# drscotthawley/signaltrain

Hardware: AMD Instinct MI355X
Metric: audio-frames/sec (train step) comp_4c 8192-sample windows @ 1/2/4/8 GPUs (higher is better)
Workload: dtype f32; 1 GPU; comp_4c synthetic, 8192-sample windows, batch 256/GPU, fp32 (BASELINE configs[1]); window=8192, frames_per_window=25, global_batch=256, parallelism=dp1

## Files before the change

### signaltrain_amd/csrc/st_api.hip

```cpp
#include <hip/hip_runtime.h>
#include <stdarg.h>
#include <stdio.h>
#include <string.h>
#include <math.h>
#include <mutex>
#include <set>
#include <utility>
#include "st_common.h"
#include "st_gemm.h"
#include "st_gemm_planes.h"
#include "st_gemm_tn.h"
#include "st_gemm16.h"
#include "st_misc.h"
#include "st_ae.h"
#include "st_ae_wide.h"
#include "st_ae_split.h"
#include "st_ae32.h"
#include "st_dp.h"
#include "st_feed.h"

static thread_local char g_err[512] = "";
int st_fail(int code, const char* fmt, ...)
{
    va_list ap; va_start(ap, fmt); vsnprintf(g_err, sizeof(g_err), fmt, ap); va_end(ap);
// ... 130 lines not shown
static int g_dbg = 0;
extern "C" int st_set_debug(int v) { g_dbg = v; return ST_OK; }
namespace sta { extern __device__ unsigned long long g_ae_stage_cycles[32]; }
extern "C" int st_debug_read_stage_cycles(unsigned long long* out32);
static int g_dp_inline = 1;
static int g_ae_save = 1;
static int g_ae_split = -1;
static int g_ae32 = 1;
static int g_pl_bf16 = 0;
static int g_wg_split = 0;
static int g_pl_dgrad = 0;
static int g_pl_shape = 3;
static int g_g16 = 1;
static int g_g16_bk = 64;
static int g_g16_dma = 0;
static int g_g16_abl = 0;
static int g_g16_split = 0;
static int g_nt128 = 1;
static int g_tn128 = 1;
static int g_tn_bk = 32;
static int g_tn_fm = 3;
static int g_g16_crop = 15;
static int g_frs_nt = 1;
static int g_xt = 0;
static const int NORM_E_PARTIALS = 32;
static const int NORM_E_MAX = 4096;
static int g_wide_pair = 1;
static int g_wide_direct = 1;
static int g_wide_dvp = 1;
static int g_nt_mi = 0;
static int g_an_bk = 32;
static int g_bk = 16;
static int g_wg_mode_set(int v);
static int g_wsplit_max = 16, g_wsplit_div = 200, g_an_waves = 4, g_syn_split = 3, g_frs_split = 3, g_wide_fused = 1, g_wsplit_half = 0;
extern "C" int st_set_tuning(int bk)
{
#ifdef ST_DIAG
    if (bk >= 96800 && bk < 96928) { g_g16_abl = bk - 96800; return ST_OK; }
#else
    if ((bk >= 96800 && bk < 96928) || (bk >= 9680 && bk < 9690)) return st_fail(ST_ERR_ARG, "st_set_tuning(%d): timing-only ablation, needs a -DST_DIAG build", bk);
#endif
    if (bk >= 9970 && bk < 9980) { g_wide_direct = bk - 9970; return ST_OK; }
    if (bk >= 9960) { g_wide_pair = bk - 9960; return ST_OK; }
    if (bk >= 9950 && bk < 9960) { g_nt128 = bk - 9950; return ST_OK; }
    if (bk >= 9900) { g_wide_dvp = bk - 9900; return ST_OK; }
    if (bk >= 9800) { g_nt_mi = bk - 9800; return ST_OK; }
    if (bk >= 9700) { g_g16_split = bk - 9700; return ST_OK; }
    if (bk >= 9690 && bk < 9700) { g_g16_dma = bk - 9690; return ST_OK; }
#ifdef ST_DIAG
    if (bk >= 9680 && bk < 9690) { g_g16_abl = bk - 9680; return ST_OK; }
#endif
    if (bk >= 9600) { const int v = bk - 9600; if (v == 32 || v == 64) g_g16_bk = v; else g_g16 = v; return ST_OK; }
    if (bk >= 9560 && bk < 9576) { g_g16_crop = bk - 9560; return ST_OK; }
    if (bk >= 9540 && bk < 9544) { g_tn_fm = bk - 9540; return ST_OK; }
    if (bk >= 9500) { const int v = bk - 9500; if (v == 16 || v == 32) g_tn_bk = v; else g_tn128 = v; return ST_OK; }
    if (bk >= 9400) { g_pl_bf16 = bk - 9400; return ST_OK; }
    if (bk >= 9300) { g_wg_split = bk - 9300; return ST_OK; }
    if (bk >= 9200) { g_pl_dgrad = bk - 9200; return ST_OK; }
    if (bk >= 9100) { g_pl_shape = bk - 9100; return ST_OK; }
    if (bk >= 9000) { g_frs_nt = bk - 9000; return ST_OK; }
    if (bk >= 8100 && bk < 8110) { g_ae32 = bk - 8100; return ST_OK; }
    if (bk == 8300 || bk == 8301) { g_dp_inline = bk - 8300; return ST_OK; }
    if (bk == 8200 || bk == 8201) { g_ae_save = bk - 8200; return ST_OK; }
    if (bk >= 8000) { g_ae_split = bk == 8002 ? -1 : bk - 8000; return ST_OK; }
    if (bk >= 7000) { g_xt = bk - 7000; return ST_OK; }
    if (bk >= 6000) { g_wsplit_half = bk - 6000; return ST_OK; }
    if (bk >= 5000) { g_wide_fused = bk - 5000; return ST_OK; }
    if (bk >= 4000) { g_frs_split = bk - 4000; return (g_frs_split >= 1 && g_frs_split <= 6) ? ST_OK : st_fail(ST_ERR_ARG, "frames split must be 1..6"); }
    if (bk >= 3000) { g_syn_split = bk - 3000; return ST_OK; }
    if (bk >= 2000) { g_an_waves = bk - 2000; return ST_OK; }
    if (bk >= 1000) { g_wsplit_div = bk - 1000; return ST_OK; }
    if (bk >= 200) { g_wsplit_max = bk - 200; return ST_OK; }
    if (bk >= 100) return g_wg_mode_set(bk - 100);
    if (bk != 16 && bk != 32) return st_fail(ST_ERR_ARG, "bk must be 16 or 32"); g_bk = bk; g_an_bk = bk; return ST_OK;
}
#define ST_TUNING_LIST(X) X(g_dbg, 0) X(g_ae_split, -1) X(g_ae_save, 1) X(g_dp_inline, 1) X(g_pl_bf16, 0) X(g_wg_split, 0) X(g_pl_dgrad, 0) X(g_pl_shape, 3) X(g_g16, 1) X(g_g16_bk, 64) X(g_g16_dma, 0) \
    X(g_g16_abl, 0) X(g_g16_split, 0) X(g_nt128, 1) X(g_tn128, 1) X(g_tn_bk, 32) X(g_frs_nt, 1) X(g_xt, 0) X(g_wide_pair, 1) X(g_wide_dvp, 1) X(g_nt_mi, 0) X(g_an_bk, 32) \
    X(g_bk, 16) X(g_wsplit_max, 16) X(g_wsplit_div, 200) X(g_an_waves, 4) X(g_syn_split, 3) X(g_frs_split, 3) X(g_wide_fused, 1) X(g_wsplit_half, 0) X(g_wg_mode, 0) X(g_ae32, 1) X(g_wide_direct, 1) X(g_tn_fm, 3) X(g_g16_crop, 15)
static int g_wg_mode = 0;
extern "C" int st_get_tuning(int* out, int n)
{
    int i = 0;
#define X(v_, d_) if (out && i < n) out[i] = v_; ++i;
    ST_TUNING_LIST(X)
#undef X
    return i;
}
extern "C" int st_tuning_defaults(int* out, int n)
{
    int i = 0;
#define X(v_, d_) if (out && i < n) out[i] = d_; ++i;
    ST_TUNING_LIST(X)
#undef X
    return i;
}
extern "C" int st_reset_tuning(void)
{
#define X(v_, d_) v_ = d_;
    ST_TUNING_LIST(X)
#undef X
    return ST_OK;
}
static inline int gemm_ht(int prec) { return (prec == ST_PREC_BF16 || prec == ST_PREC_BF16_ALL) ? 1 : ((prec == ST_PREC_F16 || prec == ST_PREC_F16_ALL) ? 2 : (prec == ST_PREC_F32X3 ? 3 : 0)); }
static inline int ae_ht(int prec) { return prec == ST_PREC_BF16_ALL ? 1 : (prec == ST_PREC_F16_ALL ? 2 : 0); }
static inline float loss_scale_of(const st_dims* d) { return d->loss_scale > 0.f ? d->loss_scale : 1.0f; }
#define ST_GEMM_BK(BK_, W_, ...) do { const int ht_ = gemm_ht(d->prec); \
// ... 345 lines not shown
    return ola_loss_impl(d, frs, x, y_true, y_hat, dsyn, 0, loss_partial, stream);
}

static int synthesis_dgrad_impl(const st_dims* d, const float* dsyn, bool padded, const float* Sfold, float* dAA, void* stream)
{
    const int KP = st_kp_of(d->F);
    const stg::RowMap ms = synth_live(d);
    const int R = ms.rows(d->B);
    stg::PlainNT bl{Sfold, KP, d->N, d->N, stg::all_frames(1)};
    stg::StoreC ep{dAA, R, KP, KP, (size_t)d->B * d->OT * KP, ms};
    const int ns = R >= 4096 ? 1 : synth_split(R);
    if (padded) {
        stg::FramedNT<true> al{dsyn, d->y, d->H, d->N, R, d->N, 1.0f, ms};
        stg::NTWork wk;
        if (use_nt128(d, R, KP) && stg::ntw_dgrad(wk, ms, d->B, d->H, d->N, d->N, d->y, d->F, KP, ns, num_cus())) {
            const stg::NTRows ra = stg::ntrows_frame_major(dsyn, (unsigned)(d->y + 2 * d->N), (unsigned)d->H, ms, d->B, R);
            const stg::NTRows rb = wk.col_h ? stg::NTRows{Sfold, (unsigned)((KP / 2) * d->N), (unsigned)d->N, stg::rowmap_magic(d->F - 1), d->F - 1, 0, 2 * (d->F - 1)}
                                            : stg::NTRows{Sfold, (unsigned)d->N, 0u, 0u, 1, 0, KP};
            const stg::StoreSlab es{dAA, R, KP, KP, (size_t)d->B * d->OT * KP, stg::frame_major(ms, d->B)};
            ST_TRY(stg::launch_nt128(ra, rb, es, wk, st_stream(stream)));
        }
        else if (R >= 4096) ST_GEMM(4, al, bl, ep, R, KP, d->N, ns, st_stream(stream));
        else if (gemm_ht(d->prec) == 0 && (g_nt_mi & 4)) stg::launch<2, 16, 2>(al, bl, ep, R, KP, d->N, ns, st_stream(stream), g_dbg);
        else ST_GEMM(2, al, bl, ep, R, KP, d->N, ns, st_stream(stream));
    } else {
        stg::FramedNT<false> al{dsyn, d->y, d->H, d->N, R, d->N, 1.0f, ms};
        if (R >= 4096) ST_GEMM(4, al, bl, ep, R, KP, d->N, ns, st_stream(stream)); else ST_GEMM(2, al, bl, ep, R, KP, d->N, ns, st_stream(stream));
    }
    ST_LAUNCHED("synthesis_dgrad");
    return ST_OK;
}
extern "C" int st_synthesis_dgrad(const st_dims* d, const float* dsyn, const float* Sfold, float* dAA, void* stream)
{
    ST_TRY(check_dims(d)); ST_REQ(dsyn && Sfold && dAA, "st_synthesis_dgrad: null pointer");
    return synthesis_dgrad_impl(d, dsyn, false, Sfold, dAA, stream);
}

static bool use_tn128(const st_dims* d, bool padded)
{
    const int ht = gemm_ht(d->prec);
    return g_tn128 && padded && (ht == 0 || (ht == 3 && !g_wg_split)) && d->N % 256 == 0 && g_wg_mode == 0;
}
struct TNFrameMajor { stg::TNOperand a, b; stg::RowMap map; stg::FrameTrim trim; bool on; };
static TNFrameMajor tn_frame_major(const stg::TNOperand& ta, const stg::TNOperand& tb, const stg::RowMap& live, int B, int H, int Ntaps, int pad, int Ls, bool enable)
{
    TNFrameMajor f; f.on = enable && B >= 2 && fm_div_exact(live.Tv * B, B); f.a = ta; f.b = tb; f.map = live; f.trim = stg::FrameTrim{}; f.trim.on = 0;
    if (!f.on) return f;
    f.a = stg::TNOperand{ta.base + (size_t)live.t_lo * ta.S2, ta.S2, ta.S1};
    f.b = stg::TNOperand{tb.base + (size_t)live.t_lo * tb.S2, tb.S2, tb.S1};
    f.map.Tv = B; f.map.t_lo = 0; f.map.magic = stg::rowmap_magic(B); f.map.fm = 0;
    f.trim = stg::frame_trim(live, B, H, Ntaps, pad, Ls);
    return f;
}
static int wgrad_tn128(const st_dims* d, const stg::TNOperand& ta, const stg::TNOperand& tb, const float* zeros, const stg::RowMap& map, int R,
                       float* ws, int ns, stm::NyqJob* nyq, void* stream, const stg::FrameTrim* trim)
{
    const int KP = st_kp_of(d->F);
    const int mh = (d->N / 2) / 128;
    float* part = ws + (size_t)ns * KP * d->N;
    int P = 0;
    const unsigned c0 = (unsigned)(d->F - 1), c1 = (unsigned)(KP / 2 + d->F - 1);
    if (g_tn_bk == 16) ST_TRY((stg::launch_tn128<16>(ta, tb, zeros, map, R, d->N, mh, (unsigned)(KP / 2), d->N, ws, d->N, (size_t)KP * d->N, ns, st_stream(stream), part, c0, c1, &P, trim)));
    else ST_TRY((stg::launch_tn128<32>(ta, tb, zeros, map, R, d->N, mh, (unsigned)(KP / 2), d->N, ws, d->N, (size_t)KP * d->N, ns, st_stream(stream), part, c0, c1, &P, trim)));
    nyq->part = part; nyq->P = P; nyq->on = 1;
    return ST_OK;
}
static int synthesis_wgrad_impl(const st_dims* d, const float* AA, const float* dsyn, bool padded, float* ws,
                                float* gSr, float* gSi, float* norm_partial, void* stream, int* defer_slabs = nullptr, stm::NyqJob* defer_nyq = nullptr)
{
    const int KP = st_kp_of(d->F);
    const stg::RowMap ms = synth_live(d);
    const int R = ms.rows(d->B);
    int ns = wgrad_split_tiles(R, KP, d->N);
    stm::NyqJob nyq{}; nyq.on = 0;
    const stg::TNOperand ta{AA, (unsigned)(d->OT * KP), (unsigned)KP}, tb{dsyn, (unsigned)(d->y + 2 * d->N), (unsigned)d->H};
    if (use_tn128(d, padded) && stg::tn128_fits(ta, tb, dsyn, ms, d->N, d->N, (size_t)d->B * d->OT * KP, (size_t)d->B * (d->y + 2 * d->N))) {
        ns = tn_split(R, d->N);
        const TNFrameMajor fm = tn_frame_major(ta, tb, ms, d->B, d->H, d->N, d->N, d->y, (g_tn_fm & 1) != 0);
        ST_TRY(wgrad_tn128(d, fm.a, fm.b, dsyn, fm.map, R, ws, ns, &nyq, stream, &fm.trim));
    } else {
        stg::PlainTN al{AA, R, KP, KP, ms};
        stg::StoreC ep{ws, KP, d->N, d->N, (size_t)KP * d->N, stg::all_frames(1)};
        if (padded) { stg::FramedTN<true> bl{dsyn, d->y, d->H, d->N, R, d->N, 1.0f, ms}; ST_GEMM_WG(al, bl, ep, KP, d->N, R, ns, st_stream(stream)); }
        else { stg::FramedTN<false> bl{dsyn, d->y, d->H, d->N, R, d->N, 1.0f, ms}; ST_GEMM_WG(al, bl, ep, KP, d->N, R, ns, st_stream(stream)); }
    }
    ST_LAUNCHED("synthesis_wgrad");
    if (defer_slabs) { *defer_slabs = ns; if (defer_nyq) *defer_nyq = nyq; return ST_OK; }
    hipLaunchKernelGGL(stm::wgrad_reduce_kernel, dim3(st_norm_partials(d)), dim3(256), 0, st_stream(stream),
                       ws, ns, gSr, gSi, norm_partial, d->N, d->F, KP, 1, 0, 2 * d->F, (float*)nullptr, nyq);
    ST_LAUNCHED("synthesis_wgrad_reduce");
    return ST_OK;
}
extern "C" int st_synthesis_wgrad(const st_dims* d, const float* AA, const float* dsyn, float* ws,
                                  float* gSr, float* gSi, float* norm_partial, void* stream)
{
    ST_TRY(check_dims(d)); ST_REQ(AA && dsyn && ws && gSr && gSi && norm_partial, "st_synthesis_wgrad: null pointer");
    return synthesis_wgrad_impl(d, AA, dsyn, false, ws, gSr, gSi, norm_partial, stream);
}


static inline int wide_half_type(const st_dims* d, int R) { (void)R; return ae_ht(d->prec); }
extern "C" int st_effective_prec(const st_dims* d)
{
    if (!d) return -1;
    if (ae_is_wide(d) && ae_ht(d->prec) && wide_half_type(d, d->B * (st_kp_of(d->F) / 2)) == 0)
        return d->prec == ST_PREC_BF16_ALL ? ST_PREC_BF16 : ST_PREC_F16;
    return d->prec;
}
#define ST_WGEMM(...) do { if (wide_ht == 1) stg::launch_half<2, 1>(__VA_ARGS__); else if (wide_ht == 2) stg::launch_half<2, 2>(__VA_ARGS__); \
                           else stg::launch<2, 16>(__VA_ARGS__, g_dbg); } while (0)
#define ST_WGEMM_PAIR(A0_, B0_, E0_, A1_, B1_, E1_, M_, N_, K_, NS_, S_) do { \
        if (wide_ht == 1 && g_wide_pair) stg::launch_half_pair<2, 1>(A0_, B0_, E0_, A1_, B1_, E1_, M_, N_, K_, NS_, S_); \
        else if (wide_ht == 2 && g_wide_pair) stg::launch_half_pair<2, 2>(A0_, B0_, E0_, A1_, B1_, E1_, M_, N_, K_, NS_, S_); \
        else { ST_WGEMM(A0_, B0_, E0_, M_, N_, K_, NS_, S_); ST_WGEMM(A1_, B1_, E1_, M_, N_, K_, NS_, S_); } } while (0)
static int ae_wide_fwd(const st_dims* d, const Layout& L, const float* mag, const float* phs, const float* knobs,
                       const float* ae_m, const float* ae_p, float* mag_hat, float* phs_hat, float* AA, float* reg_partial,
// ... 773 lines not shown
    a.nyq = stm::NyqJob{}; a.nyq.on = 0; if (syn_nyq) a.nyq = *syn_nyq;
    a.dG16 = nullptr; a.ht = 0;
    if (w.g16) { a.dG16 = w.dG16; a.ht = gemm_ht(d->prec); a.dG = nullptr; }
    a.norm_e = nullptr;
    if (d->clip_all && a.n_red <= NORM_E_MAX) { a.norm_e = w.norm_e; w.n_norm_e = a.n_red; }
    hipLaunchKernelGGL(stm::post_ae_kernel, dim3(a.n_red + a.n_polar + (syn_slabs > 0 ? st_norm_partials(d) : 0)), dim3(256), 0, st_stream(stream), a);
    ST_LAUNCHED("post_ae");
    return ST_OK;
}
static int backward_p1(const st_dims* d, const Layout& L, const float* params, float* grads,
                       const float* knobs, const float* g_mag_hat, const float* g_mag, float reg_coef, WS& w, void* stream)
{
    int syn_slabs = 0; stm::NyqJob syn_nyq{}; syn_nyq.on = 0;
    ST_TRY(backward_syn(d, L, grads, w, stream, &syn_slabs, &syn_nyq));
    return backward_ae(d, L, params, grads, knobs, g_mag_hat, g_mag, reg_coef, w, stream, syn_slabs, &syn_nyq);
}
static int backward_p2(const st_dims* d, const Layout& L, float* grads, const float* x, WS& w, void* stream, float* stage = nullptr, int stage_bf16 = 0)
{
    (void)x;
    if (w.g16) {
        const stg::RowMap ma = stg::live_frames(d->T, d->H, d->N, d->N, d->L);
        const int R = ma.rows(d->B), KP = st_kp_of(d->F), ns = g16_wsplit(d, R);
        ST_TRY(wgrad16(d, w.dG16, (unsigned)(d->T * KP), w.xp16, (unsigned)(d->L + 2 * d->N), ma, R, w.wg, ns, stream, 0, -1, (g_g16_crop & 8) ? d->L : 0));
        ST_LAUNCHED("analysis_wgrad");
        stm::NyqJob nq{}; nq.on = 0;
        hipLaunchKernelGGL(stm::wgrad_reduce_kernel, dim3(st_norm_partials(d)), dim3(256), 0, st_stream(stream),
                           w.wg, ns, grads + L.offs[0], grads + L.offs[1], w.norm_a, d->N, d->F, KP, 0, 0, 2 * d->F, stage, nq, 0, stage_bf16);
        ST_LAUNCHED("analysis_wgrad_reduce");
        return ST_OK;
    }
    return analysis_wgrad_impl(d, w.dG, w.xp, true, 1.0f, w.wg, grads + L.offs[0], grads + L.offs[1], w.norm_a, stream, -1, stage, stage_bf16);
}
static int analysis_wgrad_half(const st_dims* d, const Layout& L, float* grads, WS& w, int half, float* stage, int stage_bf16, stm::NyqJob* nyq_io, void* stream)
{
    const int KP = st_kp_of(d->F), F = d->F, N = d->N, m0 = half ? KP / 2 : 0;
    const stg::RowMap ma = stg::live_frames(d->T, d->H, d->N, d->N, d->L);
    const int R = ma.rows(d->B);
    const int room = (int)((st_wgrad_ws_floats(d) - (size_t)64 * 2 * N) / ((size_t)KP * N));
    const int per = stm::nyq_blocks(N) / 2;
    int ns;
    const stg::TNOperand ta{w.dG + m0, (unsigned)(d->T * KP), (unsigned)KP}, tb{w.xp, (unsigned)(d->L + 2 * d->N), (unsigned)d->H};
    if (w.g16) {
        const int tiles = ((KP / 2 + 127) / 128) * (N / 128);
        ns = g_g16_split > 0 ? g_g16_split : (2 * num_cus()) / (tiles > 0 ? tiles : 1);
        if (ns > R / 128) ns = R / 128; if (ns > room) ns = room; if (ns < 1) ns = 1;
        ST_TRY(wgrad16(d, w.dG16, (unsigned)(d->T * KP), w.xp16, (unsigned)(d->L + 2 * d->N), ma, R, w.wg, ns, stream, m0, KP / 2, (g_g16_crop & 8) ? d->L : 0));
        if (!half) { *nyq_io = stm::NyqJob{}; nyq_io->on = 0; }
    } else if (use_tn128(d, true) && stg::tn128_fits(ta, tb, w.xp, ma, N / 2, N, (size_t)d->B * d->T * KP, (size_t)d->B * (d->L + 2 * d->N))) {
        const int mh = (N / 2) / 128, tiles = mh * (N / 128);
        ns = num_cus() / (tiles > 0 ? tiles : 1); if (ns > 16) ns = 16; if (ns > R / 64) ns = R / 64; if (ns > room) ns = room; if (ns < 1) ns = 1;
        float* part = w.wg + (size_t)room * KP * N;
        int P = 0;
        const TNFrameMajor fm = tn_frame_major(ta, tb, ma, d->B, d->H, N, N, d->L, (g_tn_fm & 2) != 0);
        if (g_tn_bk == 16) ST_TRY((stg::launch_tn128<16>(fm.a, fm.b, w.xp, fm.map, R, N / 2, mh, (unsigned)(KP / 2), N, w.wg + (size_t)m0 * N, N, (size_t)KP * N, ns, st_stream(stream),
                                                          half ? nullptr : part, (unsigned)(F - 1), (unsigned)(KP / 2 + F - 1), &P, &fm.trim)));
        else ST_TRY((stg::launch_tn128<32>(fm.a, fm.b, w.xp, fm.map, R, N / 2, mh, (unsigned)(KP / 2), N, w.wg + (size_t)m0 * N, N, (size_t)KP * N, ns, st_stream(stream),
                                            half ? nullptr : part, (unsigned)(F - 1), (unsigned)(KP / 2 + F - 1), &P, &fm.trim)));
        if (!half) { nyq_io->part = part; nyq_io->P = P; nyq_io->on = 1; }
    } else {
        ST_LAUNCHED("analysis_wgrad");
        if (!half) { *nyq_io = stm::NyqJob{}; nyq_io->on = 0; }
        return analysis_wgrad_impl(d, w.dG, w.xp, true, 1.0f, w.wg, grads + L.offs[0], grads + L.offs[1], w.norm_a, stream, half, stage, stage_bf16);
    }
    ST_LAUNCHED("analysis_wgrad");
    hipLaunchKernelGGL(stm::wgrad_reduce_kernel, dim3(F + per), dim3(256), 0, st_stream(stream),
                       w.wg, ns, grads + L.offs[0], grads + L.offs[1], w.norm_a, N, F, KP, 0, half * F, F, stage, *nyq_io, half * per, stage_bf16);
    ST_LAUNCHED("analysis_wgrad_reduce");
    return ST_OK;
}
static int backward_impl(const st_dims* d, const Layout& L, const float* params, float* grads, const float* x,
                         const float* knobs, const float* g_mag_hat, const float* g_mag, float reg_coef, WS& w, void* stream)
{
    ST_TRY(backward_p1(d, L, params, grads, knobs, g_mag_hat, g_mag, reg_coef, w, stream));
    return backward_p2(d, L, grads, x, w, stream);
}

extern "C" int st_model_fwd(const st_dims* d, const float* params, const float* x, const float* knobs,
                            float* y_hat, float* mag, float* mag_hat, void* ws, int save_for_backward, void* stream)
{
    Layout L; ST_TRY(make_layout(d, &L));
    ST_REQ(params && x && (knobs || d->K == 0) && ws, "st_model_fwd: null pointer");
    if (!knobs) knobs = params;
    WS w; carve(d, ws, &w);
    return forward_impl(d, L, params, x, knobs, nullptr, y_hat, mag, mag_hat, w, save_for_backward != 0, stream);
}

extern "C" int st_model_bwd(const st_dims* d, const float* params, float* grads, const float* x, const float* knobs,
                            const float* g_y_hat, const float* g_mag_hat, const float* g_mag, void* ws, void* stream)
{
    Layout L; ST_TRY(make_layout(d, &L));
    ST_REQ(params && grads && x && (knobs || d->K == 0) && g_y_hat && ws, "st_model_bwd: null pointer");
    if (!knobs) knobs = params;
    WS w; carve(d, ws, &w);
    ST_TRY(pad_scale(g_y_hat, w.dsyn, d->B, d->y, d->N, 2.0f, stream));
    return backward_impl(d, L, params, grads, x, knobs, g_mag_hat, g_mag, 0.0f, w, stream);
}

__global__ void knob_grad_kernel(const float* __restrict__ Wm, const float* __restrict__ gbm, const float* __restrict__ Wp, const float* __restrict__ gbp,
                                 const int K, float* __restrict__ out)
{
    const int k = threadIdx.x;
    if (k >= K) return;
    float s = 0.f, t = 0.f;
    for (int o = 0; o < 16; ++o) { s += Wm[o * (16 + K) + 16 + k] * gbm[o]; t += Wp[o * (16 + K) + 16 + k] * gbp[o]; }
    out[k] = s + t;
}
extern "C" int st_model_knob_grad(const st_dims* d, const float* params, float* grads_scratch, const float* x, const float* knobs,
                                  const float* g_y_hat, const float* g_mag_hat, const float* g_mag, void* ws, float* g_knobs, void* stream)
{
    Layout L; ST_TRY(make_layout(d, &L));
// ... 620 lines not shown
```

### signaltrain_amd/csrc/st_gemm_tn.h

```cpp
#pragma once
#include "st_gemm.h"

namespace stg {

struct TNJob {
    const float* base;
    unsigned a0, b0;
    unsigned SA1, SA2, SB1, SB2;
    unsigned magic; int Tv, t_lo;
    int K;
    unsigned zero;
    int mh; unsigned mstride;
    float* nyq_out; unsigned nyq_c0, nyq_c1; int nyq_P, Nc, nsplit;
    int trim, fB; unsigned char fa[64], fb[64];
};
struct FrameTrim { int on, B; unsigned char fa[64], fb[64]; };
static inline FrameTrim frame_trim(const RowMap& live, int B, int H, int Ntaps, int pad, int Ls)
{
    FrameTrim f; f.on = (Ntaps % 128 == 0 && Ntaps / 128 <= 64 && live.Tv <= 255) ? 1 : 0; f.B = B;
    for (int j = 0; j < 64; ++j) { f.fa[j] = 0; f.fb[j] = (unsigned char)(live.Tv <= 255 ? live.Tv : 255); }
    if (!f.on) return f;
    for (int j = 0; j < Ntaps / 128; ++j) {
        const int n0 = 128 * j;
        int a = 0, b = live.Tv;
        while (a < b && H * (live.t_lo + a) + n0 + 127 < pad) ++a;
        while (b > a && H * (live.t_lo + b - 1) + n0 >= pad + Ls) --b;
        f.fa[j] = (unsigned char)a; f.fb[j] = (unsigned char)b;
    }
    return f;
}

__device__ __forceinline__ void nyq_partial(const TNJob& j, const int p)
{
    if (p >= j.nyq_P) return;
    const int per = (j.K + j.nyq_P - 1) / j.nyq_P, k0 = p * per, k1 = (k0 + per < j.K) ? k0 + per : j.K;
    for (int n4 = threadIdx.x; n4 < j.Nc / 4; n4 += 256) {
        float4 s0 = make_float4(0.f, 0.f, 0.f, 0.f), s1 = s0;
        for (int kb = k0; kb < k1; kb += 8) {
            float a0[8], a1[8]; float4 x[8];
#pragma unroll
            for (int u = 0; u < 8; ++u) {
                const int k = kb + u < k1 ? kb + u : k1 - 1;
                const unsigned w = __umulhi((unsigned)k, j.magic), t = (unsigned)j.t_lo + ((unsigned)k - w * (unsigned)j.Tv);
                const float* arow = j.base + j.a0 + (size_t)w * j.SA1 + (size_t)t * j.SA2;
                a0[u] = kb + u < k1 ? arow[j.nyq_c0] : 0.f; a1[u] = kb + u < k1 ? arow[j.nyq_c1] : 0.f;
                x[u] = *reinterpret_cast<const float4*>(j.base + j.b0 + (size_t)w * j.SB1 + (size_t)t * j.SB2 + 4 * n4);
            }
#pragma unroll
            for (int u = 0; u < 8; ++u) {
                s0.x = __builtin_fmaf(a0[u], x[u].x, s0.x); s0.y = __builtin_fmaf(a0[u], x[u].y, s0.y); s0.z = __builtin_fmaf(a0[u], x[u].z, s0.z); s0.w = __builtin_fmaf(a0[u], x[u].w, s0.w);
                s1.x = __builtin_fmaf(a1[u], x[u].x, s1.x); s1.y = __builtin_fmaf(a1[u], x[u].y, s1.y); s1.z = __builtin_fmaf(a1[u], x[u].z, s1.z); s1.w = __builtin_fmaf(a1[u], x[u].w, s1.w);
            }
        }
        float* o = j.nyq_out + (size_t)p * 2 * j.Nc + 4 * n4;
        *reinterpret_cast<float4*>(o) = s0;
        *reinterpret_cast<float4*>(o + j.Nc) = s1;
    }
}

template <int BKT>
__global__ void __launch_bounds__(256)
gemm_tn128_kernel(const TNJob j, float* __restrict__ out, const int ldo, const size_t slab, const int ksplit)
{
    constexpr int TS = BKT * 128;
    constexpr int NP = BKT / 8;
    constexpr int KS = BKT / 2;
    extern __shared__ __attribute__((aligned(16))) float tn_lds[];
    float* const As = tn_lds;
    float* const Bs = tn_lds + 2 * TS;

    const int tid = threadIdx.x, lane = tid & 63, wave = tid >> 6, wm = wave >> 1, wn = wave & 1;
    if ((int)blockIdx.z >= j.nsplit) { nyq_partial(j, (int)(blockIdx.y * gridDim.x + blockIdx.x)); return; }
    int tbx, tby, tbz; xcd_tile(tbx, tby, tbz, j.nsplit);
    const unsigned rowA = (unsigned)(tby % j.mh) * 128u + (unsigned)(tby / j.mh) * j.mstride;
    const unsigned colB = (unsigned)tbx * 128u;
    int k_begin = tbz * ksplit;
    int k_end = (k_begin + ksplit < j.K) ? k_begin + ksplit : j.K;
    if (j.trim) {
        const int lo = (int)j.fa[tbx] * j.fB, hi = (int)j.fb[tbx] * j.fB;
        const int per = ((hi - lo + j.nsplit - 1) / j.nsplit + BKT - 1) / BKT * BKT;
        k_begin = lo + tbz * per;
        k_end = (k_begin + per < hi) ? k_begin + per : hi;
    }

    const int c4 = tid & 31, kr = tid >> 5;
    const unsigned la = 4u * (j.a0 + rowA + 4u * (unsigned)c4), lb = 4u * (j.b0 + colB + 4u * (unsigned)c4), lz = 4u * (j.zero + 4u * (unsigned)c4);
    const unsigned sa1 = 4u * j.SA1, sa2 = 4u * j.SA2, sb1 = 4u * j.SB1, sb2 = 4u * j.SB2;
    float4 ra[NP], rb[NP];
    auto ld = [&](const unsigned byte_off) { return *reinterpret_cast<const float4*>(reinterpret_cast<const char*>(j.base) + byte_off); };
    auto gload = [&](const int kt) {
#pragma unroll
        for (int p = 0; p < NP; ++p) {
            const int k = kt + kr + 8 * p;
            const unsigned kc = (unsigned)(k < j.K ? k : j.K - 1);
            const unsigned b = __umulhi(kc, j.magic);
            const unsigned t = (unsigned)j.t_lo + kc - __umul24(b, (unsigned)j.Tv);
            const unsigned oa = __umul24(b, sa1) + __umul24(t, sa2) + la;
            const unsigned ob = __umul24(b, sb1) + __umul24(t, sb2) + lb;
            const unsigned live = (unsigned)((k - j.K) >> 31);
            ra[p] = ld((oa & live) | (lz & ~live));
            rb[p] = ld(ob);
        }
    };
    auto lstore = [&](const int buf) {
        float* as = As + buf * TS + kr * 128 + 4 * c4;
        float* bs = Bs + buf * TS + kr * 128 + 4 * c4;
#pragma unroll
        for (int p = 0; p < NP; ++p) {
            *reinterpret_cast<float4*>(as + p * 8 * 128) = ra[p];
            *reinterpret_cast<float4*>(bs + p * 8 * 128) = rb[p];
        }
    };

    f32x16 acc[2][2];
#pragma unroll
    for (int mi = 0; mi < 2; ++mi)
#pragma unroll
        for (int nj = 0; nj < 2; ++nj)
#pragma unroll
            for (int i = 0; i < 16; ++i) acc[mi][nj][i] = 0.f;

    const int h = lane >> 5, l31 = lane & 31;
    if (k_begin < k_end) {
        gload(k_begin);
        lstore(0);
        __syncthreads();
        int cur = 0;
        const int a_off = h * 128 + wm * 64 + 2 * l31;
        const int b_off = h * 128 + wn * 64 + 2 * l31;
        for (int kt = k_begin; kt < k_end; kt += BKT) {
            const bool more = kt + BKT < k_end;
            gload(more ? kt + BKT : kt);
            __builtin_amdgcn_sched_barrier(0);
            const float* as = As + cur * TS + a_off;
            const float* bs = Bs + cur * TS + b_off;
            float2 fa[2][2], fb[2][2];
            auto frag = [&](const int pr, const int buf) {
#pragma unroll
                for (int u = 0; u < 2; ++u) {
                    fa[buf][u] = *reinterpret_cast<const float2*>(as + (2 * pr + u) * 256);
                    fb[buf][u] = *reinterpret_cast<const float2*>(bs + (2 * pr + u) * 256);
                }
            };
            frag(0, 0);
#pragma unroll
            for (int pr = 0; pr < KS / 2; ++pr) {
                if (pr + 1 < KS / 2) frag(pr + 1, (pr + 1) & 1);
#pragma unroll
                for (int u = 0; u < 2; ++u) {
                    const float2 a = fa[pr & 1][u], b = fb[pr & 1][u];
                    acc[0][0] = __builtin_amdgcn_mfma_f32_32x32x2f32(a.x, b.x, acc[0][0], 0, 0, 0);
                    acc[0][1] = __builtin_amdgcn_mfma_f32_32x32x2f32(a.x, b.y, acc[0][1], 0, 0, 0);
                    acc[1][0] = __builtin_amdgcn_mfma_f32_32x32x2f32(a.y, b.x, acc[1][0], 0, 0, 0);
                    acc[1][1] = __builtin_amdgcn_mfma_f32_32x32x2f32(a.y, b.y, acc[1][1], 0, 0, 0);
                }
            }
            __builtin_amdgcn_sched_group_barrier(0x100, 2, 0);
#pragma unroll
            for (int pr = 0; pr < KS / 2; ++pr) {
                if (pr + 1 < KS / 2) __builtin_amdgcn_sched_group_barrier(0x100, 2, 0);
                __builtin_amdgcn_sched_group_barrier(0x008, 8, 0);
            }
            __builtin_amdgcn_sched_barrier(0);
            lstore(cur ^ 1);
            __syncthreads();
            cur ^= 1;
        }
    }
    float* o = out + (size_t)tbz * slab + (size_t)(rowA + wm * 64) * ldo + colB + wn * 64 + 2 * l31;
#pragma unroll
    for (int i = 0; i < 16; ++i) {
        const int r = 2 * d_row(i, lane);
#pragma unroll
        for (int mi = 0; mi < 2; ++mi)
            *reinterpret_cast<float2*>(o + (size_t)(r + mi) * ldo) = make_float2(acc[mi][0][i], acc[mi][1][i]);
    }
}

struct TNOperand { const float* base; unsigned S1, S2; };
static inline bool tn128_fits(const TNOperand& A, const TNOperand& B, const float* zeros, const RowMap& map, int M, int Nc, size_t extentA, size_t extentB)
{
    if (M % 128 || Nc % 128 || map.Tv < 2) return false;
    const unsigned lim24 = 1u << 22;
    if (A.S1 >= lim24 || A.S2 >= lim24 || B.S1 >= lim24 || B.S2 >= lim24) return false;
    const float* lo = A.base < B.base ? A.base : B.base; if (zeros < lo) lo = zeros;
    const size_t lim = (size_t)1 << 30;
    return (size_t)(A.base - lo) + extentA < lim && (size_t)(B.base - lo) + extentB < lim && (size_t)(zeros - lo) + 128 < lim;
}
template <int BKT>
static inline int launch_tn128(const TNOperand& A, const TNOperand& B, const float* zeros, const RowMap& map, int K,
                               int M, int mh, unsigned mstride, int Nc, float* out, int ldo, size_t slab, int nsplit, hipStream_t s,
                               float* nyq_out = nullptr, unsigned nyq_c0 = 0, unsigned nyq_c1 = 0, int* nyq_P = nullptr, const FrameTrim* trim = nullptr)
{
    const float* lo = A.base < B.base ? A.base : B.base; if (zeros < lo) lo = zeros;
    TNJob j;
    j.base = lo; j.a0 = (unsigned)(A.base - lo); j.b0 = (unsigned)(B.base - lo); j.zero = (unsigned)(zeros - lo);
    j.SA1 = A.S1; j.SA2 = A.S2; j.SB1 = B.S1; j.SB2 = B.S2;
    j.magic = map.magic; j.Tv = map.Tv; j.t_lo = map.t_lo; j.K = K; j.mh = mh; j.mstride = mstride;
    j.trim = (trim && trim->on) ? 1 : 0; j.fB = trim ? trim->B : 0;
    for (int i = 0; i < 64; ++i) { j.fa[i] = trim ? trim->fa[i] : 0; j.fb[i] = trim ? trim->fb[i] : 0; }
    int ksplit = K;
    if (nsplit > 1) ksplit = st_round_up((K + nsplit - 1) / nsplit, BKT);
    constexpr size_t lds = (size_t)4 * BKT * 128 * sizeof(float);
    if (lds > 65536) { const int rc = ::ensure_dyn_lds((const void*)gemm_tn128_kernel<BKT>, "gemm_tn128_kernel"); if (rc) return rc; }
    const int nz = nsplit > 1 ? nsplit : 1, tiles = (Nc / 128) * (M / 128);
    j.nsplit = nz; j.Nc = Nc; j.nyq_out = nyq_out; j.nyq_c0 = nyq_c0; j.nyq_c1 = nyq_c1;
    j.nyq_P = tiles < 64 ? tiles : 64; { const int W = K / 8 > 0 ? K / 8 : 1; if (j.nyq_P > W) j.nyq_P = W; }
    if (nyq_P) *nyq_P = j.nyq_P;
    hipLaunchKernelGGL((gemm_tn128_kernel<BKT>), dim3(Nc / 128, M / 128, nz + (nyq_out ? 1 : 0)), dim3(256), lds, s, j, out, ldo, slab, ksplit);
    return 0;
}

}

namespace stg {

struct NTRows { const float* base; unsigned S1, S2, magic; int Tv, t_lo, R; };
__device__ __forceinline__ unsigned ntrows_off(const NTRows& o, const int r)
{
    const unsigned rc = (unsigned)(r < o.R ? r : o.R - 1);
    const unsigned b = o.magic ? __umulhi(rc, o.magic) : rc;
    const unsigned t = o.magic ? (unsigned)o.t_lo + (rc - b * (unsigned)o.Tv) : 0u;
    return b * o.S1 + t * o.S2;
}
static inline NTRows ntrows_frame_major(const float* base, unsigned s_window, unsigned s_frame, const RowMap& live, int B, int R)
{
    return NTRows{base + (size_t)live.t_lo * s_frame, s_frame, s_window, B > 1 ? rowmap_magic(B) : 0u, B, 0, R};
}

constexpr int NTW_MAX = 768;
struct NTWork {
    int n, nslabs;
    int col_h, col_stride;
    int kunit, kt_total;
    unsigned nyq_b[2], nyq_col[2];
    unsigned e[NTW_MAX];
};
static inline unsigned ntw_pack(int mt, int nt, int z, int zf, int kind, int k0, int kl)
{
    return (unsigned)mt | (unsigned)nt << 8 | (unsigned)z << 14 | (unsigned)zf << 16 | (unsigned)kind << 18 | (unsigned)k0 << 19 | (unsigned)kl << 25;
}

struct StoreSlab {
    float* out; int M, Nc, ld; size_t slab; RowMap map;
    __device__ void operator()(const int z, const int m0, const int n0, const f32x16 (&acc)[2]) const {
        const int lane = threadIdx.x & 63;
        float* o = out + (size_t)z * slab;
#pragma unroll
        for (int i = 0; i < 16; ++i) {
            const int row = m0 + d_row(i, lane);
            if (row < M) {
                float* orow = o + (size_t)map.full(row) * ld;
#pragma unroll
                for (int j = 0; j < 2; ++j) {
                    const int col = n0 + 32 * j + (lane & 31);
                    if (col < Nc) orow[col] = acc[j][i];
                }
            }
        }
    }
};

// ... 39 lines not shown
    constexpr int NP = 4;
    extern __shared__ __attribute__((aligned(16))) float nt_lds[];
    float* const As = nt_lds;
    float* const Bs = nt_lds + 2 * TS;
    const int tid = threadIdx.x, lane = tid & 63, wave = tid >> 6, wm = wave >> 1, wn = wave & 1;
    const unsigned ent = wk.e[blockIdx.x];
    const int m_blk = (int)(ent & 255u) * 128, n_blk = (int)((ent >> 8) & 63u) * 128, tbz = (int)((ent >> 14) & 3u), zf = (int)((ent >> 16) & 3u);
    const int k_begin = (int)((ent >> 19) & 63u) * wk.kunit * BKT;
    int k_end = k_begin + (int)(ent >> 25) * wk.kunit * BKT;
    if (k_end > wk.kt_total * BKT) k_end = wk.kt_total * BKT;
    if ((ent >> 18) & 1u) { nt128_nyquist(ra, rb, epi, wk, m_blk, k_begin, k_end); return; }

    const int lr = tid >> 3, lk = (tid & 7) * 4;
    unsigned ao[NP], bo[NP];
#pragma unroll
    for (int p = 0; p < NP; ++p) {
        ao[p] = 4u * (ntrows_off(ra, m_blk + lr + 32 * p) + (unsigned)lk);
        bo[p] = 4u * (ntrows_off(rb, n_blk + lr + 32 * p) + (unsigned)lk);
    }
    f32x4 va[NP], vb[NP];
    auto gload = [&](const int kt) {
        const char* pa = reinterpret_cast<const char*>(ra.base) + 4 * (size_t)kt;
        const char* pb = reinterpret_cast<const char*>(rb.base) + 4 * (size_t)kt;
#pragma unroll
        for (int p = 0; p < NP; ++p) {
            va[p] = *reinterpret_cast<const f32x4*>(pa + ao[p]);
            vb[p] = *reinterpret_cast<const f32x4*>(pb + bo[p]);
        }
    };
    auto lstore = [&](const int buf) {
        float* as = As + buf * TS + lr * LD + lk;
        float* bs = Bs + buf * TS + lr * LD + lk;
#pragma unroll
        for (int p = 0; p < NP; ++p) {
            *reinterpret_cast<f32x4*>(as + p * 32 * LD) = va[p];
            *reinterpret_cast<f32x4*>(bs + p * 32 * LD) = vb[p];
        }
    };
    f32x16 acc[2][2];
#pragma unroll
    for (int mi = 0; mi < 2; ++mi)
#pragma unroll
        for (int nj = 0; nj < 2; ++nj)
#pragma unroll
            for (int i = 0; i < 16; ++i) acc[mi][nj][i] = 0.f;

    if (k_begin < k_end) {
        gload(k_begin);
        lstore(0);
        __syncthreads();
        int cur = 0;
        const int h = lane >> 5, l31 = lane & 31;
        const int a_off = (wm * 64 + l31) * LD + 16 * h, b_off = (wn * 64 + l31) * LD + 16 * h;
        for (int kt = k_begin; kt < k_end; kt += BKT) {
            const bool more = kt + BKT < k_end;
            gload(more ? kt + BKT : kt);
            __builtin_amdgcn_sched_barrier(0);
            const float* as = As + cur * TS + a_off;
            const float* bs = Bs + cur * TS + b_off;
            f32x4 fa[2][2][2], fb[2][2][2];
#pragma unroll
            for (int hf = 0; hf < 2; ++hf)
#pragma unroll
                for (int x = 0; x < 2; ++x)
#pragma unroll
                    for (int q = 0; q < 2; ++q) {
                        fa[hf][x][q] = *reinterpret_cast<const f32x4*>(as + x * 32 * LD + 8 * hf + 4 * q);
                        fb[hf][x][q] = *reinterpret_cast<const f32x4*>(bs + x * 32 * LD + 8 * hf + 4 * q);
                    }
#pragma unroll
            for (int hf = 0; hf < 2; ++hf)
#pragma unroll
                for (int q = 0; q < 2; ++q)
#pragma unroll
                    for (int e = 0; e < 4; ++e) {
                        const float a0 = fa[hf][0][q][e], a1 = fa[hf][1][q][e];
                        const float b0 = fb[hf][0][q][e], b1 = fb[hf][1][q][e];
                        acc[0][0] = __builtin_amdgcn_mfma_f32_32x32x2f32(a0, b0, acc[0][0], 0, 0, 0);
                        acc[0][1] = __builtin_amdgcn_mfma_f32_32x32x2f32(a0, b1, acc[0][1], 0, 0, 0);
                        acc[1][0] = __builtin_amdgcn_mfma_f32_32x32x2f32(a1, b0, acc[1][0], 0, 0, 0);
                        acc[1][1] = __builtin_amdgcn_mfma_f32_32x32x2f32(a1, b1, acc[1][1], 0, 0, 0);
                    }
            lstore(cur ^ 1);
            __builtin_amdgcn_sched_group_barrier(0x100, 8, 0);
#pragma unroll
            for (int i = 0; i < 8; ++i) { __builtin_amdgcn_sched_group_barrier(0x008, 4, 0); __builtin_amdgcn_sched_group_barrier(0x100, 1, 0); }
            __builtin_amdgcn_sched_group_barrier(0x008, 16, 0);
#pragma unroll
            for (int i = 0; i < 8; ++i) { __builtin_amdgcn_sched_group_barrier(0x008, 2, 0); __builtin_amdgcn_sched_group_barrier(0x200, 1, 0); }
            __builtin_amdgcn_sched_barrier(0);
            __syncthreads();
            cur ^= 1;
        }
    }
    const int c_blk = wk.col_h ? (n_blk % wk.col_h) + (n_blk / wk.col_h) * wk.col_stride : n_blk;
#pragma unroll
    for (int mi = 0; mi < 2; ++mi) epi(tbz, m_blk + wm * 64 + 32 * mi, c_blk + wn * 64, acc[mi]);
    if (zf > 0 && zf < wk.nslabs) {
#pragma unroll
        for (int mi = 0; mi < 2; ++mi)
#pragma unroll
            for (int nj = 0; nj < 2; ++nj)
#pragma unroll
                for (int i = 0; i < 16; ++i) acc[mi][nj][i] = 0.f;
        for (int z = zf; z < wk.nslabs; ++z) {
#pragma unroll
            for (int mi = 0; mi < 2; ++mi) epi(z, m_blk + wm * 64 + 32 * mi, c_blk + wn * 64, acc[mi]);
        }
    }
}

static inline void ntw_tile_frames(const RowMap& live, int B, int R, int mt, int& f0, int& f1)
{
    const int r0 = mt * 128, r1 = (r0 + 128 < R ? r0 + 128 : R) - 1;
    f0 = live.t_lo + r0 / B; f1 = live.t_lo + r1 / B;
}
static inline void ntw_live_taps(int f0, int f1, int H, int N, int pad, int Ls, int& lo, int& hi)
{
    lo = pad - H * f1; if (lo < 0) lo = 0;
    hi = pad + Ls - H * f0; if (hi > N) hi = N;
    if (hi <= lo) { lo = 0; hi = N; }
}
static inline void ntw_push(NTWork& w, int mt, int nt, int z, int zf, int kind, int k0, int kl)
{
    w.e[w.n++] = ntw_pack(mt, nt, z, zf, kind, k0, kl);
}
static inline void ntw_xcd_order(NTWork& w)
{
    unsigned tmp[NTW_MAX];
    const int T = w.n, q = T >> 3, r = T & 7;
    for (int L = 0; L < T; ++L) { const int j = L & 7; tmp[L] = w.e[j * q + (j < r ? j : r) + (L >> 3)]; }
    for (int L = 0; L < T; ++L) w.e[L] = tmp[L];
}
static inline double ntw_cost(int wgs, int ktiles, int ncus) { return (double)((wgs + ncus - 1) / ncus) * (6.0 + 2.35 * (double)ktiles); }
static inline bool ntw_rounds_ok(int wgs, int ncus) { const int r = (wgs + ncus - 1) / ncus; return r <= 1 || (double)wgs >= 0.85 * (double)r * (double)ncus; }
static inline bool ntw_header(NTWork& w, int nslabs, int ktiles)
{
    w.n = 0; w.nslabs = nslabs; w.col_h = 0; w.col_stride = 0; w.nyq_b[0] = w.nyq_b[1] = w.nyq_col[0] = w.nyq_col[1] = 0u;
    w.kunit = (ktiles + 63) / 64; w.kt_total = ktiles;
    return nslabs >= 1 && nslabs <= 3 && ktiles >= 1 && (ktiles + w.kunit - 1) / w.kunit <= 127;
}
static inline bool ntw_frames(NTWork& w, const RowMap& live, int B, int H, int N, int pad, int Ls, int K, int nslabs, int ncus)
{
    const int R = live.rows(B), MT = (R + 127) / 128;
// ... 74 lines not shown
```

Measured before the change: 10.67 million frames/s.

## Software-pipeline TN128 wgrad GEMM with interleaved LDS stores and prefetch

Adds a pipelined variant of the TN128 weight-gradient kernel. It interleaves LDS fragment reads, stores of the next tile and global loads two tiles ahead within the MFMA loop, with a single barrier per tile. It also adds a uniform-address path that hoists per-row offset math when frame counts divide the tile depth. The kernel gains a waves-per-EU hint, and compile-time ablation switches are added for timing. The aim is to hide load and barrier latency behind MFMA, at the cost of extra register pressure and more complex scheduling.

Measured after the change: 10.96 million frames/s (median of 6 runs). +2.7%, better.

```diff
diff --git a/signaltrain_amd/csrc/st_api.hip b/signaltrain_amd/csrc/st_api.hip
--- a/signaltrain_amd/csrc/st_api.hip
+++ b/signaltrain_amd/csrc/st_api.hip
@@ -206,6 +206,7 @@
 #endif
     if (bk >= 9600) { const int v = bk - 9600; if (v == 32 || v == 64) g_g16_bk = v; else g_g16 = v; return ST_OK; }
     if (bk >= 9560 && bk < 9576) { g_g16_crop = bk - 9560; return ST_OK; }
+    if (bk == 9580 || bk == 9581) { g_tn128 = bk == 9580 ? 2 : 1; return ST_OK; }
     if (bk >= 9540 && bk < 9544) { g_tn_fm = bk - 9540; return ST_OK; }
     if (bk >= 9500) { const int v = bk - 9500; if (v == 16 || v == 32) g_tn_bk = v; else g_tn128 = v; return ST_OK; }
     if (bk >= 9400) { g_pl_bf16 = bk - 9400; return ST_OK; }
@@ -657,6 +658,8 @@
     f.trim = stg::frame_trim(live, B, H, Ntaps, pad, Ls);
     return f;
 }
+#define ST_TN128(...) do { if (g_tn_bk == 16) { if (g_tn128 == 2) ST_TRY((stg::launch_tn128<16, false>(__VA_ARGS__))); else ST_TRY((stg::launch_tn128<16, true>(__VA_ARGS__))); } \
+                           else if (g_tn128 == 2) ST_TRY((stg::launch_tn128<32, false>(__VA_ARGS__))); else ST_TRY((stg::launch_tn128<32, true>(__VA_ARGS__))); } while (0)
 static int wgrad_tn128(const st_dims* d, const stg::TNOperand& ta, const stg::TNOperand& tb, const float* zeros, const stg::RowMap& map, int R,
                        float* ws, int ns, stm::NyqJob* nyq, void* stream, const stg::FrameTrim* trim)
 {
@@ -665,8 +668,7 @@
     float* part = ws + (size_t)ns * KP * d->N;
     int P = 0;
     const unsigned c0 = (unsigned)(d->F - 1), c1 = (unsigned)(KP / 2 + d->F - 1);
-    if (g_tn_bk == 16) ST_TRY((stg::launch_tn128<16>(ta, tb, zeros, map, R, d->N, mh, (unsigned)(KP / 2), d->N, ws, d->N, (size_t)KP * d->N, ns, st_stream(stream), part, c0, c1, &P, trim)));
-    else ST_TRY((stg::launch_tn128<32>(ta, tb, zeros, map, R, d->N, mh, (unsigned)(KP / 2), d->N, ws, d->N, (size_t)KP * d->N, ns, st_stream(stream), part, c0, c1, &P, trim)));
+    ST_TN128(ta, tb, zeros, map, R, d->N, mh, (unsigned)(KP / 2), d->N, ws, d->N, (size_t)KP * d->N, ns, st_stream(stream), part, c0, c1, &P, trim);
     nyq->part = part; nyq->P = P; nyq->on = 1;
     return ST_OK;
 }
@@ -1546,10 +1548,8 @@
         float* part = w.wg + (size_t)room * KP * N;
         int P = 0;
         const TNFrameMajor fm = tn_frame_major(ta, tb, ma, d->B, d->H, N, N, d->L, (g_tn_fm & 2) != 0);
-        if (g_tn_bk == 16) ST_TRY((stg::launch_tn128<16>(fm.a, fm.b, w.xp, fm.map, R, N / 2, mh, (unsigned)(KP / 2), N, w.wg + (size_t)m0 * N, N, (size_t)KP * N, ns, st_stream(stream),
-                                                          half ? nullptr : part, (unsigned)(F - 1), (unsigned)(KP / 2 + F - 1), &P, &fm.trim)));
-        else ST_TRY((stg::launch_tn128<32>(fm.a, fm.b, w.xp, fm.map, R, N / 2, mh, (unsigned)(KP / 2), N, w.wg + (size_t)m0 * N, N, (size_t)KP * N, ns, st_stream(stream),
-                                            half ? nullptr : part, (unsigned)(F - 1), (unsigned)(KP / 2 + F - 1), &P, &fm.trim)));
+        ST_TN128(fm.a, fm.b, w.xp, fm.map, R, N / 2, mh, (unsigned)(KP / 2), N, w.wg + (size_t)m0 * N, N, (size_t)KP * N, ns, st_stream(stream),
+                 half ? nullptr : part, (unsigned)(F - 1), (unsigned)(KP / 2 + F - 1), &P, &fm.trim);
         if (!half) { nyq_io->part = part; nyq_io->P = P; nyq_io->on = 1; }
     } else {
         ST_LAUNCHED("analysis_wgrad");
diff --git a/signaltrain_amd/csrc/st_gemm_tn.h b/signaltrain_amd/csrc/st_gemm_tn.h
--- a/signaltrain_amd/csrc/st_gemm_tn.h
+++ b/signaltrain_amd/csrc/st_gemm_tn.h
@@ -1,5 +1,10 @@
 #pragma once
 #include "st_gemm.h"
+
+#ifndef ST_G128_ABLATE
+#define ST_G128_ABLATE 0
+#endif
+#define ST_G128_KEEP4(v_) asm volatile("" :: "v"((v_)[0]), "v"((v_)[1]), "v"((v_)[2]), "v"((v_)[3]))
 
 namespace stg {
 
@@ -58,8 +63,8 @@
     }
 }
 
-template <int BKT>
-__global__ void __launch_bounds__(256)
+template <int BKT, bool PIPE = false, bool UNI = false>
+__global__ void __launch_bounds__(256) __attribute__((amdgpu_waves_per_eu(1, 2)))
 gemm_tn128_kernel(const TNJob j, float* __restrict__ out, const int ldo, const size_t slab, const int ksplit)
 {
     constexpr int TS = BKT * 128;
@@ -88,28 +93,30 @@
     const unsigned sa1 = 4u * j.SA1, sa2 = 4u * j.SA2, sb1 = 4u * j.SB1, sb2 = 4u * j.SB2;
     float4 ra[NP], rb[NP];
     auto ld = [&](const unsigned byte_off) { return *reinterpret_cast<const float4*>(reinterpret_cast<const char*>(j.base) + byte_off); };
+    auto gload_pass = [&](const int kt, const int p) {
+        const int k = kt + kr + 8 * p;
+        const unsigned kc = (unsigned)(k < j.K ? k : j.K - 1);
+        const unsigned b = __umulhi(kc, j.magic);
+        const unsigned t = (unsigned)j.t_lo + kc - __umul24(b, (unsigned)j.Tv);
+        const unsigned oa = __umul24(b, sa1) + __umul24(t, sa2) + la;
+        const unsigned ob = __umul24(b, sb1) + __umul24(t, sb2) + lb;
+        const unsigned live = (unsigned)((k - j.K) >> 31);
+        ra[p] = ld((oa & live) | (lz & ~live));
+        rb[p] = ld(ob);
+    };
     auto gload = [&](const int kt) {
 #pragma unroll
-        for (int p = 0; p < NP; ++p) {
-            const int k = kt + kr + 8 * p;
-            const unsigned kc = (unsigned)(k < j.K ? k : j.K - 1);
-            const unsigned b = __umulhi(kc, j.magic);
-            const unsigned t = (unsigned)j.t_lo + kc - __umul24(b, (unsigned)j.Tv);
-            const unsigned oa = __umul24(b, sa1) + __umul24(t, sa2) + la;
-            const unsigned ob = __umul24(b, sb1) + __umul24(t, sb2) + lb;
-            const unsigned live = (unsigned)((k - j.K) >> 31);
-            ra[p] = ld((oa & live) | (lz & ~live));
-            rb[p] = ld(ob);
-        }
+        for (int p = 0; p < NP; ++p) gload_pass(kt, p);
+    };
+    auto lstore_pass = [&](const int buf, const int p) {
+        float* as = As + buf * TS + kr * 128 + 4 * c4;
+        float* bs = Bs + buf * TS + kr * 128 + 4 * c4;
+        *reinterpret_cast<float4*>(as + p * 8 * 128) = ra[p];
+        *reinterpret_cast<float4*>(bs + p * 8 * 128) = rb[p];
     };
     auto lstore = [&](const int buf) {
-        float* as = As + buf * TS + kr * 128 + 4 * c4;
-        float* bs = Bs + buf * TS + kr * 128 + 4 * c4;
-#pragma unroll
-        for (int p = 0; p < NP; ++p) {
-            *reinterpret_cast<float4*>(as + p * 8 * 128) = ra[p];
-            *reinterpret_cast<float4*>(bs + p * 8 * 128) = rb[p];
-        }
+#pragma unroll
+        for (int p = 0; p < NP; ++p) lstore_pass(buf, p);
     };
 
     f32x16 acc[2][2];
@@ -121,16 +128,85 @@
             for (int i = 0; i < 16; ++i) acc[mi][nj][i] = 0.f;
 
     const int h = lane >> 5, l31 = lane & 31;
-    if (k_begin < k_end) {
+    if constexpr (PIPE) {
+        constexpr int PAIRS = KS / 2;
+        static_assert(PAIRS % 2 == 0 && NP + 1 <= PAIRS - 1, "fragment buffers alternate by pair; stores and loads sit before the barrier");
+        const int ntiles = (k_end - k_begin + BKT - 1) / BKT;
+        if (ntiles > 0) {
+            const int k_last = k_begin + (ntiles - 1) * BKT;
+            unsigned ua[UNI ? NP : 1], ub[UNI ? NP : 1];
+            if constexpr (UNI) {
+#pragma unroll
+                for (int p = 0; p < NP; ++p) { ua[p] = la + (unsigned)(kr + 8 * p) * sa2; ub[p] = lb + (unsigned)(kr + 8 * p) * sb2; }
+            }
+            auto gl = [&](const int kt, const int p) {
+                if constexpr (UNI) {
+                    const unsigned b = __umulhi((unsigned)kt, j.magic), t0 = (unsigned)j.t_lo + (unsigned)kt - b * (unsigned)j.Tv;
+                    ra[p] = ld(b * sa1 + t0 * sa2 + ua[p]);
+                    rb[p] = ld(b * sb1 + t0 * sb2 + ub[p]);
+                } else gload_pass(kt, p);
+            };
+            const int a_off = h * 128 + wm * 64 + 2 * l31;
+            const int b_off = h * 128 + wn * 64 + 2 * l31;
+            float2 fa[2][2], fb[2][2];
+            auto frag = [&](const int stage, const int pr, const int buf) {
+                const float* as = As + stage * TS + a_off;
+                const float* bs = Bs + stage * TS + b_off;
+#pragma unroll
+                for (int u = 0; u < 2; ++u) {
+                    fa[buf][u] = *reinterpret_cast<const float2*>(as + (2 * pr + u) * 256);
+                    fb[buf][u] = *reinterpret_cast<const float2*>(bs + (2 * pr + u) * 256);
+                }
+            };
+            auto mfma8 = [&](const int buf) {
+#pragma unroll
+                for (int u = 0; u < 2; ++u) {
+                    const float2 a = fa[buf][u], b = fb[buf][u];
+                    acc[0][0] = __builtin_amdgcn_mfma_f32_32x32x2f32(a.x, b.x, acc[0][0], 0, 0, 0);
+                    acc[0][1] = __builtin_amdgcn_mfma_f32_32x32x2f32(a.x, b.y, acc[0][1], 0, 0, 0);
+                    acc[1][0] = __builtin_amdgcn_mfma_f32_32x32x2f32(a.y, b.x, acc[1][0], 0, 0, 0);
+                    acc[1][1] = __builtin_amdgcn_mfma_f32_32x32x2f32(a.y, b.y, acc[1][1], 0, 0, 0);
+                }
+            };
+#pragma unroll
+            for (int p = 0; p < NP; ++p) gl(k_begin, p);
+            lstore(0);
+#pragma unroll
+            for (int p = 0; p < NP; ++p) gl(ntiles > 1 ? k_begin + BKT : k_begin, p);
+            __syncthreads();
+            frag(0, 0, 0);
+            int cur = 0;
+            for (int i = 0; i < ntiles; ++i) {
+                const int k2 = k_begin + (i + 2) * BKT, kn = k2 < k_last ? k2 : k_last;
+                __builtin_amdgcn_sched_barrier(0);
+#pragma unroll
+                for (int pr = 0; pr < PAIRS - 1; ++pr) {
+                    frag(cur, pr + 1, (pr + 1) & 1);
+                    if (pr < NP) lstore_pass(cur ^ 1, pr);
+                    if (pr >= 1 && pr <= NP) gl(kn, pr - 1);
+                    mfma8(pr & 1);
+                    __builtin_amdgcn_sched_barrier(0);
+                }
+                __syncthreads();
+                frag(cur ^ 1, 0, 0);
+                mfma8(1);
+                __builtin_amdgcn_sched_barrier(0);
+                cur ^= 1;
+            }
+        }
+    } else if (k_begin < k_end) {
         gload(k_begin);
         lstore(0);
         __syncthreads();
         int cur = 0;
         const int a_off = h * 128 + wm * 64 + 2 * l31;
         const int b_off = h * 128 + wn * 64 + 2 * l31;
+        float2 abl_f[4];
+#pragma unroll
+        for (int u = 0; u < 4; ++u) abl_f[u] = (ST_G128_ABLATE & 2) ? *reinterpret_cast<const float2*>(As + a_off + u * 256) : make_float2(0.f, 0.f);
         for (int kt = k_begin; kt < k_end; kt += BKT) {
             const bool more = kt + BKT < k_end;
-            gload(more ? kt + BKT : kt);
+            if (!(ST_G128_ABLATE & 8)) gload(more ? kt + BKT : kt);
             __builtin_amdgcn_sched_barrier(0);
             const float* as = As + cur * TS + a_off;
             const float* bs = Bs + cur * TS + b_off;
@@ -138,6 +214,7 @@
             auto frag = [&](const int pr, const int buf) {
 #pragma unroll
                 for (int u = 0; u < 2; ++u) {
+                    if (ST_G128_ABLATE & 2) { fa[buf][u] = abl_f[(2 * buf + u) & 3]; fb[buf][u] = abl_f[(2 * buf + u + 1) & 3]; continue; }
                     fa[buf][u] = *reinterpret_cast<const float2*>(as + (2 * pr + u) * 256);
                     fb[buf][u] = *reinterpret_cast<const float2*>(bs + (2 * pr + u) * 256);
                 }
@@ -162,8 +239,12 @@
                 __builtin_amdgcn_sched_group_barrier(0x008, 8, 0);
             }
             __builtin_amdgcn_sched_barrier(0);
-            lstore(cur ^ 1);
-            __syncthreads();
+            if (!(ST_G128_ABLATE & 4)) lstore(cur ^ 1);
+            else {
+#pragma unroll
+                for (int p = 0; p < NP; ++p) { asm volatile("" :: "v"(ra[p].x), "v"(ra[p].y), "v"(ra[p].z), "v"(ra[p].w)); asm volatile("" :: "v"(rb[p].x), "v"(rb[p].y), "v"(rb[p].z), "v"(rb[p].w)); }
+            }
+            if (!(ST_G128_ABLATE & 1)) __syncthreads();
             cur ^= 1;
         }
     }
@@ -187,7 +268,12 @@
     const size_t lim = (size_t)1 << 30;
     return (size_t)(A.base - lo) + extentA < lim && (size_t)(B.base - lo) + extentB < lim && (size_t)(zeros - lo) + 128 < lim;
 }
-template <int BKT>
+static inline bool tn128_uniform(const RowMap& map, int K, int bkt, const FrameTrim* trim)
+{
+    if (map.Tv % bkt || K % bkt) return false;
+    return !(trim && trim->on) || trim->B % bkt == 0;
+}
+template <int BKT, bool PIPE = false>
 static inline int launch_tn128(const TNOperand& A, const TNOperand& B, const float* zeros, const RowMap& map, int K,
                                int M, int mh, unsigned mstride, int Nc, float* out, int ldo, size_t slab, int nsplit, hipStream_t s,
                                float* nyq_out = nullptr, unsigned nyq_c0 = 0, unsigned nyq_c1 = 0, int* nyq_P = nullptr, const FrameTrim* trim = nullptr)
@@ -202,12 +288,15 @@
     int ksplit = K;
     if (nsplit > 1) ksplit = st_round_up((K + nsplit - 1) / nsplit, BKT);
     constexpr size_t lds = (size_t)4 * BKT * 128 * sizeof(float);
-    if (lds > 65536) { const int rc = ::ensure_dyn_lds((const void*)gemm_tn128_kernel<BKT>, "gemm_tn128_kernel"); if (rc) return rc; }
+    static_assert(lds <= 65536, "the Nyquist side workgroups share a CU with a GEMM workgroup: 2 x 64 KB of the 160");
     const int nz = nsplit > 1 ? nsplit : 1, tiles = (Nc / 128) * (M / 128);
     j.nsplit = nz; j.Nc = Nc; j.nyq_out = nyq_out; j.nyq_c0 = nyq_c0; j.nyq_c1 = nyq_c1;
     j.nyq_P = tiles < 64 ? tiles : 64; { const int W = K / 8 > 0 ? K / 8 : 1; if (j.nyq_P > W) j.nyq_P = W; }
     if (nyq_P) *nyq_P = j.nyq_P;
-    hipLaunchKernelGGL((gemm_tn128_kernel<BKT>), dim3(Nc / 128, M / 128, nz + (nyq_out ? 1 : 0)), dim3(256), lds, s, j, out, ldo, slab, ksplit);
+    const dim3 grid(Nc / 128, M / 128, nz + (nyq_out ? 1 : 0));
+    if (!PIPE) hipLaunchKernelGGL((gemm_tn128_kernel<BKT>), grid, dim3(256), lds, s, j, out, ldo, slab, ksplit);
+    else if (tn128_uniform(map, K, BKT, trim)) hipLaunchKernelGGL((gemm_tn128_kernel<BKT, PIPE, PIPE>), grid, dim3(256), lds, s, j, out, ldo, slab, ksplit);
+    else hipLaunchKernelGGL((gemm_tn128_kernel<BKT, PIPE, false>), grid, dim3(256), lds, s, j, out, ldo, slab, ksplit);
     return 0;
 }
 
@@ -353,9 +442,12 @@
         int cur = 0;
         const int h = lane >> 5, l31 = lane & 31;
         const int a_off = (wm * 64 + l31) * LD + 16 * h, b_off = (wn * 64 + l31) * LD + 16 * h;
+        f32x4 abl_f[4];
+#pragma unroll
+        for (int u = 0; u < 4; ++u) abl_f[u] = (ST_G128_ABLATE & 2) ? *reinterpret_cast<const f32x4*>(As + a_off + 4 * u) : f32x4{0.f, 0.f, 0.f, 0.f};
         for (int kt = k_begin; kt < k_end; kt += BKT) {
             const bool more = kt + BKT < k_end;
-            gload(more ? kt + BKT : kt);
+            if (!(ST_G128_ABLATE & 8)) gload(more ? kt + BKT : kt);
             __builtin_amdgcn_sched_barrier(0);
             const float* as = As + cur * TS + a_off;
             const float* bs = Bs + cur * TS + b_off;
@@ -366,6 +458,7 @@
                 for (int x = 0; x < 2; ++x)
 #pragma unroll
                     for (int q = 0; q < 2; ++q) {
+                        if (ST_G128_ABLATE & 2) { fa[hf][x][q] = abl_f[(2 * x + q) & 3]; fb[hf][x][q] = abl_f[(2 * x + q + 1) & 3]; continue; }
                         fa[hf][x][q] = *reinterpret_cast<const f32x4*>(as + x * 32 * LD + 8 * hf + 4 * q);
                         fb[hf][x][q] = *reinterpret_cast<const f32x4*>(bs + x * 32 * LD + 8 * hf + 4 * q);
                     }
@@ -382,7 +475,11 @@
                         acc[1][0] = __builtin_amdgcn_mfma_f32_32x32x2f32(a1, b0, acc[1][0], 0, 0, 0);
                         acc[1][1] = __builtin_amdgcn_mfma_f32_32x32x2f32(a1, b1, acc[1][1], 0, 0, 0);
                     }
-            lstore(cur ^ 1);
+            if (!(ST_G128_ABLATE & 4)) lstore(cur ^ 1);
+            else {
+#pragma unroll
+                for (int p = 0; p < NP; ++p) { ST_G128_KEEP4(va[p]); ST_G128_KEEP4(vb[p]); }
+            }
             __builtin_amdgcn_sched_group_barrier(0x100, 8, 0);
 #pragma unroll
             for (int i = 0; i < 8; ++i) { __builtin_amdgcn_sched_group_barrier(0x008, 4, 0); __builtin_amdgcn_sched_group_barrier(0x100, 1, 0); }
@@ -390,7 +487,7 @@
 #pragma unroll
             for (int i = 0; i < 8; ++i) { __builtin_amdgcn_sched_group_barrier(0x008, 2, 0); __builtin_amdgcn_sched_group_barrier(0x200, 1, 0); }
             __builtin_amdgcn_sched_barrier(0);
-            __syncthreads();
+            if (!(ST_G128_ABLATE & 1)) __syncthreads();
             cur ^= 1;
         }
     }
```
